# oriolfornes/ExplaiNN

Hardware: AMD Instinct MI355X
Metric: sequences/sec (fwd+bwd), 200bp one-hot, 300 units, batch 1024 (higher is better)
Workload: dtype f32

## Files before the change

### explainn_amd/csrc/convpool.hip

```cpp
#include <cstdlib>
#include <type_traits>

#include "common.h"

typedef __attribute__((ext_vector_type(8))) __bf16 cbf16x8;
typedef float cf32x16 __attribute__((ext_vector_type(16)));
typedef uint32_t cu32x4 __attribute__((ext_vector_type(4)));

template <int KS, int UT> struct cpm_state {
    cu32x4 Wr[UT][KS][3];
    cf32x16 acc[3][UT];
    float best[UT][16];
    uint32_t arg[UT][16];
    cu32x4 bop[3][KS];
    uint32_t xs[3], nx[2];
    uint32_t gw[4], mw[3];
    uint32_t smask[UT][16];
    uint32_t so, so4;
    uint32_t r1, r5;
};
struct cpm_args {
    const uint32_t* pk2; const uint32_t* nmask; float* ext; uint8_t* idx;
    int n, Bs, PW, NW, t0, b, kh; uint32_t tbase;
    uint32_t row1, row5;
    __amdgpu_buffer_rsrc_t rext, ridx;
};
__device__ __forceinline__ constexpr int cpm_role(int i) { return i == 0 ? 0 : ((i & 1) ? 1 : 2); }

template <int KS, int UT>
__device__ __forceinline__ void cpm_fetch(cpm_state<KS, UT>& S, const cpm_args& A, int w) {
    const int p0 = POOLW * w, wi = p0 >> 4, ni = p0 >> 5;
#pragma unroll
    for (int i = 0; i < 4; ++i) S.gw[i] = A.pk2[(size_t)min(wi + i, A.PW - 1) * A.Bs + A.b];
#pragma unroll
    for (int i = 0; i < 3; ++i) S.mw[i] = A.nmask[(size_t)min(ni + i, A.NW - 1) * A.Bs + A.b];
}
template <int KS, int UT>
__device__ __forceinline__ void cpm_window_words(cpm_state<KS, UT>& S, const cpm_args& A, int w) {
    const int p0 = POOLW * w;
    const int sh = (p0 & 15) * 2, nsh = p0 & 31;
    const uint32_t w0 = __funnelshift_r(S.gw[0], S.gw[1], sh), w1 = __funnelshift_r(S.gw[1], S.gw[2], sh),
                   w2 = __funnelshift_r(S.gw[2], S.gw[3], sh);
    S.xs[0] = __funnelshift_r(w0, w1, 4 * A.kh); S.xs[1] = __funnelshift_r(w1, w2, 4 * A.kh);
    S.xs[2] = w2 >> (4 * A.kh);
    const uint32_t nm0 = __funnelshift_r(S.mw[0], S.mw[1], nsh), nm1 = __funnelshift_r(S.mw[1], S.mw[2], nsh);
    S.nx[0] = __funnelshift_r(nm0, nm1, 2 * A.kh); S.nx[1] = nm1 >> (2 * A.kh);
    cpm_fetch(S, A, w + 1);
}
template <int KS, int UT, int I, int KSI, int BUF>
__device__ __forceinline__ void cpm_operand(cpm_state<KS, UT>& S, const cpm_args& A) {
    typedef __attribute__((address_space(3))) cu32x4 lds_u4;
    typedef __attribute__((address_space(3))) char lds_char;
    constexpr int off = 2 * I + 8 * KSI, wd = off >> 5, o = off & 31;
    constexpr int noff = I + 4 * KSI, nwd = noff >> 5, no = noff & 31;
    uint32_t cs, ns;
    if constexpr (o + 4 <= 32) {
        if constexpr (o >= 4) cs = S.xs[wd] >> (o - 4); else cs = S.xs[wd] << (4 - o);
    } else {
        cs = __funnelshift_r(S.xs[wd], S.xs[wd + 1], o) << 4;
    }
    if constexpr (no + 2 <= 32) {
        if constexpr (no >= 8) ns = S.nx[nwd] >> (no - 8); else ns = S.nx[nwd] << (8 - no);
    } else {
        ns = __funnelshift_r(S.nx[nwd], S.nx[nwd + 1], no) << 8;
    }
    const uint32_t a = ((cs & 0xF0u) | A.tbase) | (ns & 0x300u);
    S.bop[BUF][KSI] = *reinterpret_cast<const lds_u4*>((const lds_char*)(size_t)a);
}
template <int KS, int UT, bool IDX, int PI, int ROLE>
__device__ __forceinline__ void cpm_update_cmp(cpm_state<KS, UT>& S, int t, int r, unsigned long long& gt) {
    const float v = S.acc[ROLE][t][r];
    if (PI == 0) {
        S.best[t][r] = v;
    } else if (IDX) {
        asm volatile("v_cmp_gt_f32_e64 %0, %1, %2" : "=s"(gt) : "v"(v), "v"(S.best[t][r]));
    } else {
        float bv = S.best[t][r];
        asm volatile("v_max_f32 %0, %0, %1" : "+v"(bv) : "v"(v));
        S.best[t][r] = bv;
    }
}
template <int KS, int UT, bool IDX, int PI, int ROLE>
__device__ __forceinline__ void cpm_update_sel(cpm_state<KS, UT>& S, int t, int r, unsigned long long gt) {
    if (PI != 0 && IDX) {
        const float v = S.acc[ROLE][t][r];
        float bv = S.best[t][r];
        uint32_t av = PI == 1 ? 0u : S.arg[t][r];
        asm volatile("v_cndmask_b32_e64 %0, %0, %1, %2" : "+v"(bv) : "v"(v), "s"(gt));
        if (PI == 1) asm volatile("v_cndmask_b32_e64 %0, 0, 1, %1" : "=v"(av) : "s"(gt));
        else asm volatile("v_cndmask_b32_e64 %0, %0, %1, %2" : "+v"(av) : "n"(PI), "s"(gt));
        S.best[t][r] = bv; S.arg[t][r] = av;
    }
}
template <int KS, int UT, bool IDX, int PI, int ROLE>
__device__ __forceinline__ void cpm_update(cpm_state<KS, UT>& S, int t, int r) {
    unsigned long long gt = 0;
    cpm_update_cmp<KS, UT, IDX, PI, ROLE>(S, t, r, gt);
    asm volatile("s_nop 1");
    cpm_update_sel<KS, UT, IDX, PI, ROLE>(S, t, r, gt);
}
template <int KS, int UT, bool IDX>
__device__ __forceinline__ void cpm_store(cpm_state<KS, UT>& S, const cpm_args& A, int t, int r) {
    __builtin_amdgcn_raw_buffer_store_b32(__float_as_uint(S.best[t][r]) ^ S.smask[t][r], A.rext, (int)S.so4, 0, 0);
    if (IDX) __builtin_amdgcn_raw_buffer_store_b8((uint8_t)S.arg[t][r], A.ridx, (int)S.so, 0, 0);
    if (IDX) S.so += (r & 3) == 3 ? S.r5 : S.r1;
    S.so4 += (r & 3) == 3 ? 4u * S.r5 : 4u * S.r1;
}
#define CPM_OOB 0xFFFFFF00u

__device__ __forceinline__ uint32_t cpm_store_origin(const cpm_args& A, int w) {
    return (uint32_t)((4 * A.kh * A.n + w) * A.Bs + A.b);
}

#define CPM_GUARD 2
template <int K0, int K1, typename F>
__device__ __forceinline__ void cpm_static_for(F&& f) {
    if constexpr (K0 < K1) {
        f(std::integral_constant<int, K0>{});
        cpm_static_for<K0 + 1, K1>(f);
    }
}
template <int KS, int UT, int I> struct cpm_sched {
    static constexpr int NM = 3 * KS * UT;
    static constexpr int T0 = (UT + 1) / 2;
    static constexpr int NX = I == 6 ? 1 : 0, NG = KS, NE = 16 * UT;
    static constexpr int NS0 = I == 0 ? 16 * T0 : 0;
    static constexpr int NS1 = I == 1 ? 16 * (UT - T0) : 0;
    static constexpr int WX = 12, WG = 5, WE = (I == 1) ? 1 : 3, WS = 9;
    static constexpr int TOT = NX * WX + NG * WG + NE * WE + (NS0 + NS1) * WS;
    static constexpr int NU = NX + NG + NS1 + NE + NS0;
    static constexpr int E0 = NX + NG + NS1;
    static constexpr int weight(int k) {
        return k < NX ? WX : k < NX + NG ? WG : k < E0 ? WS : k < E0 + NE ? WE : WS;
    }
    static constexpr int slot(int k) {
        int cum = 0;
        for (int j = 0; j < k; ++j) cum += weight(j);
        int sl = (cum * NM) / (TOT > 0 ? TOT : 1);
        if (k >= E0 && sl < CPM_GUARD) sl = CPM_GUARD < NM ? CPM_GUARD : NM - 1;
        return sl < NM ? sl : NM - 1;
    }
    static constexpr int first_unit(int m) {
        int k = 0;
        while (k < NU && slot(k) < m) ++k;
        return k;
    }
};

template <int KS, int UT, bool IDX, int I>
__device__ __forceinline__ void cpm_position(cpm_state<KS, UT>& S, const cpm_args& A, int w) {
    typedef cpm_sched<KS, UT, I> SC;
    constexpr int NM = SC::NM;
    constexpr int RM = cpm_role(I), RN = cpm_role((I + 1) % POOLW), RP = cpm_role((I + POOLW - 1) % POOLW);
    constexpr int PI = (I + POOLW - 1) % POOLW;
    unsigned long long gt[3] = {0, 0, 0};
    cpm_static_for<0, NM>([&](auto mc) {
        constexpr int m = decltype(mc)::value;
        constexpr int pc = 2 - m / (KS * UT), ks = (m / UT) % KS, t = m % UT;
        if constexpr (m < UT)
            asm volatile("v_mfma_f32_32x32x16_bf16 %0, %1, %2, 0"
                         : "=&v"(S.acc[RM][t]) : "a"(S.Wr[t][ks][pc]), "a"(S.bop[RM][ks]));
        else
            asm volatile("v_mfma_f32_32x32x16_bf16 %0, %1, %2, %0"
                         : "+v"(S.acc[RM][t]) : "a"(S.Wr[t][ks][pc]), "a"(S.bop[RM][ks]));
        cpm_static_for<SC::first_unit(m), SC::first_unit(m + 1)>([&](auto kc) {
            constexpr int k = decltype(kc)::value;
            if constexpr (k < SC::NX) {
                cpm_window_words(S, A, w + 1);
            } else if constexpr (k < SC::NX + SC::NG) {
                cpm_operand<KS, UT, (I + 1) % POOLW, k - SC::NX, RN>(S, A);
            } else if constexpr (k < SC::E0) {
                constexpr int e = k - SC::NX - SC::NG;
                cpm_store<KS, UT, IDX>(S, A, SC::T0 + e / 16, e % 16);
            } else if constexpr (k < SC::E0 + SC::NE) {
                constexpr int e = k - SC::E0;
                if constexpr (e == 0 && NM <= CPM_GUARD) asm volatile("s_nop 15\n\ts_nop 15" ::: "memory");
                cpm_update_cmp<KS, UT, IDX, PI, RP>(S, e / 16, e % 16, gt[e % 3]);
                if constexpr (e > 1) cpm_update_sel<KS, UT, IDX, PI, RP>(S, (e - 2) / 16, (e - 2) % 16, gt[(e - 2) % 3]);
                if constexpr (e == SC::NE - 1) {
                    cpm_update_sel<KS, UT, IDX, PI, RP>(S, (e - 1) / 16, (e - 1) % 16, gt[(e - 1) % 3]);
                    cpm_update_sel<KS, UT, IDX, PI, RP>(S, e / 16, e % 16, gt[e % 3]);
                }
            } else {
                constexpr int e = k - SC::E0 - SC::NE;
                cpm_store<KS, UT, IDX>(S, A, e / 16, e % 16);
            }
        });
        __builtin_amdgcn_sched_barrier(0);
    });
}

template <int KS, int UT, bool IDX>
__device__ __forceinline__ void cpm_window(cpm_state<KS, UT>& S, const cpm_args& A, int w) {
    cpm_position<KS, UT, IDX, 0>(S, A, w);
    cpm_position<KS, UT, IDX, 1>(S, A, w);
    cpm_position<KS, UT, IDX, 2>(S, A, w);
    cpm_position<KS, UT, IDX, 3>(S, A, w);
    cpm_position<KS, UT, IDX, 4>(S, A, w);
    cpm_position<KS, UT, IDX, 5>(S, A, w);
    cpm_position<KS, UT, IDX, 6>(S, A, w);
}

template <int KS, int UT>
__device__ __forceinline__ void cpm_load_fragments(cpm_state<KS, UT>& S, const cu32x4* wsrc) {
    cpm_static_for<0, UT * KS * 3>([&S, wsrc](auto ic) {
        constexpr int i = decltype(ic)::value;
        cu32x4& dst = S.Wr[i / (KS * 3)][(i / 3) % KS][i % 3];
        const cu32x4* src = wsrc + 64 * i;
        asm volatile("global_load_dwordx4 %0, %1, off" : "=a"(dst) : "v"(src));
    });
}

struct cpm_bn1_args {
    const unsigned long long* bm; double* G; double* m;
    const float* conv_w; const float* conv_b; const float* g1; const float* b1;
    float* rm; float* rv; int64_t* nbt;
    float* alpha; float* shift; double* mug; double* sig1; double* Gw;
    int* ticket; int* flags;
    int naux, nz;
    int U, U4, k, B, L, Lp;
};
typedef __attribute__((address_space(1))) unsigned long long bn1_gu64;
typedef __attribute__((address_space(1))) int bn1_gi32;
template <int KS, int UT> struct bn1_cfg {
    static constexpr bool big = UT == 2 && KS >= 2;
    static constexpr int TQ = big ? 16 : 4;
    static constexpr int CH = big ? 40 : 12;
};
#define BN1_NU 2
#define BN1_SPIN_TICKS 10000000ull

__device__ __forceinline__ void bn1_store(double* p, double v) {
    __hip_atomic_store((bn1_gu64*)p, (unsigned long long)__double_as_longlong(v), __ATOMIC_RELAXED,
                       __HIP_MEMORY_SCOPE_AGENT);
}

template <int BN1_TQ>
__device__ __forceinline__ void bn1_moments_job(const cpm_bn1_args& X, int job, int lane) {
    const int d = job >> 2, a = job & 3;
    const int NT = (X.B + 63) / 64, Lo = X.L - X.k + 1, K4 = 4 * X.k;
    const size_t plane = (size_t)NT * X.Lp;
    const unsigned long long* __restrict__ m0 = X.bm + (size_t)a * plane;
    long long carry[4] = {0, 0, 0, 0}, plo[4] = {0, 0, 0, 0}, phi[4] = {0, 0, 0, 0};
    const int jlo = lane - 1, jhi = lane + Lo - 1;
    for (int qb = 0; qb < X.L; qb += 64) {
        const int q = qb + lane;
        int c[4] = {0, 0, 0, 0};
        if (q + d < X.L) {
            for (int t0 = 0; t0 < NT; t0 += BN1_TQ) {
                unsigned long long x0[BN1_TQ], x1[4][BN1_TQ];
#pragma unroll
                for (int i = 0; i < BN1_TQ; ++i) {
                    const size_t o = (size_t)min(t0 + i, NT - 1) * X.Lp + q;
                    x0[i] = m0[o];
#pragma unroll
                    for (int a2 = 0; a2 < 4; ++a2) x1[a2][i] = X.bm[a2 * plane + d + o];
                }
#pragma unroll
                for (int i = 0; i < BN1_TQ; ++i)
#pragma unroll
                    for (int a2 = 0; a2 < 4; ++a2) c[a2] += (t0 + i < NT) ? __popcll(x0[i] & x1[a2][i]) : 0;
            }
        }
#pragma unroll
        for (int a2 = 0; a2 < 4; ++a2) {
            int v = c[a2];
#pragma unroll
            for (int off = 1; off < 64; off <<= 1) {
                const int y = __shfl_up(v, off, 64);
                if (lane >= off) v += y;
            }
            const int vlo = __shfl(v, jlo & 63, 64), vhi = __shfl(v, jhi & 63, 64);
            if (jlo >= qb && jlo < qb + 64) plo[a2] = carry[a2] + vlo;
            if (jhi >= qb && jhi < qb + 64) phi[a2] = carry[a2] + vhi;
            carry[a2] += __shfl(v, 63, 64);
        }
    }
    const int j = lane;
    if (j < X.k - d) {
#pragma unroll
        for (int a2 = 0; a2 < 4; ++a2) {
            const long long sj = phi[a2] - plo[a2];
            const double v = (double)sj / ((double)X.B * (double)Lo);
            const int row = a * X.k + j, col = a2 * X.k + j + d;
            bn1_store(X.G + (size_t)row * K4 + col, v);
            bn1_store(X.G + (size_t)col * K4 + row, v);
            if (row == col) bn1_store(X.m + row, v);
        }
    }
}

template <int CH>
__device__ __forceinline__ void bn1_fold_units(const cpm_bn1_args& X, const int (&us)[BN1_NU], int nu, int lane) {
    const int K4 = 4 * X.k, Lo = X.L - X.k + 1;
    const int i0 = lane, i1 = lane + 64;
    const int c0i = min(i0, K4 - 1), c1i = min(i1, K4 - 1);
    float wl[BN1_NU][2];
#pragma unroll
    for (int uu = 0; uu < BN1_NU; ++uu) {
        const int u = min(us[uu], X.U - 1);
        wl[uu][0] = X.conv_w[(size_t)u * K4 + c0i];
        wl[uu][1] = X.conv_w[(size_t)u * K4 + c1i];
    }
    const double m0 = X.m[c0i], m1 = X.m[c1i];
    double ge[BN1_NU][2], go[BN1_NU][2];
#pragma unroll
    for (int uu = 0; uu < BN1_NU; ++uu) ge[uu][0] = ge[uu][1] = go[uu][0] = go[uu][1] = 0;
    for (int cb = 0; cb < K4; cb += CH) {
        double gv[CH][2];
#pragma unroll
        for (int cc = 0; cc < CH; ++cc) {
            const int c = min(cb + cc, K4 - 1);
            gv[cc][0] = X.G[(size_t)c * K4 + c0i];
            gv[cc][1] = X.G[(size_t)c * K4 + c1i];
        }
#pragma unroll
        for (int cc = 0; cc < CH; cc += 2) {
            const int c = cb + cc;
            if (c < K4) {
#pragma unroll
                for (int uu = 0; uu < BN1_NU; ++uu) {
                    const float we = __int_as_float(__builtin_amdgcn_readlane(
                        __float_as_int(c < 64 ? wl[uu][0] : wl[uu][1]), c & 63));
                    const float wo = __int_as_float(__builtin_amdgcn_readlane(
                        __float_as_int(c + 1 < 64 ? wl[uu][0] : wl[uu][1]), (c + 1) & 63));
#pragma unroll
                    for (int h = 0; h < 2; ++h) {
                        ge[uu][h] = fma(gv[cc][h], (double)we, ge[uu][h]);
                        go[uu][h] = fma(gv[cc + 1][h], (double)wo, go[uu][h]);
                    }
                }
            }
        }
    }
#pragma unroll
    for (int uu = 0; uu < BN1_NU; ++uu) {
        if (uu >= nu) break;
        const int u = us[uu];
        if (u >= X.U) {
            if (lane == 0) { X.alpha[u] = 0.f; X.shift[u] = 0.f; }
            continue;
        }
        double mu_p[2] = {0, 0}, q_p[2] = {0, 0};
#pragma unroll
        for (int h = 0; h < 2; ++h) {
            const int i = h ? i1 : i0;
            const double gw = ge[uu][h] + go[uu][h];
            if (i < K4) {
                X.Gw[(size_t)u * K4 + i] = gw;
                mu_p[h] = fma((double)wl[uu][h], h ? m1 : m0, mu_p[h]);
                q_p[h] = fma((double)wl[uu][h], gw, q_p[h]);
            }
        }
        const double mu = wave_sum_d(mu_p[0]) + wave_sum_d(mu_p[1]);
        const double wGw = wave_sum_d(q_p[0]) + wave_sum_d(q_p[1]);
        if (lane == 0)
            bn1_fold_finish(mu, wGw, u, X.g1[u], X.b1[u], X.conv_b[u], X.rm[u], X.rv[u], X.B, Lo, X.alpha,
                            X.shift, X.mug, X.sig1, X.rm, X.rv, X.nbt);
    }
}

template <int KS, int UT>
__device__ __forceinline__ void cpm_bn1(const cpm_bn1_args& X, int id, int lane) {
    for (int job = id; job < 4 * X.k; job += X.naux) bn1_moments_job<bn1_cfg<KS, UT>::TQ>(X, job, lane);
    asm volatile("s_waitcnt vmcnt(0)" ::: "memory");
    if (lane == 0) __hip_atomic_fetch_add((bn1_gi32*)X.ticket, 1, __ATOMIC_RELAXED, __HIP_MEMORY_SCOPE_AGENT);
    const unsigned long long t0 = wall_clock64();
    while (__builtin_amdgcn_readfirstlane(
               __hip_atomic_load((bn1_gi32*)X.ticket, __ATOMIC_RELAXED, __HIP_MEMORY_SCOPE_AGENT)) < X.naux) {
        if (wall_clock64() - t0 > BN1_SPIN_TICKS) {
            if (lane == 0)
                __hip_atomic_fetch_or((bn1_gi32*)X.flags, EXPLAINN_FLAG_BN1_TIMEOUT, __ATOMIC_RELAXED,
                                      __HIP_MEMORY_SCOPE_AGENT);
            return;
        }
        __builtin_amdgcn_s_sleep(2);
    }
    __builtin_amdgcn_fence(__ATOMIC_ACQUIRE, "agent");
    for (int u0 = id; u0 < X.U4; u0 += BN1_NU * X.naux) {
        int us[BN1_NU], nu = 0;
#pragma unroll
        for (int uu = 0; uu < BN1_NU; ++uu) {
            us[uu] = u0 + uu * X.naux;
            if (us[uu] < X.U4) nu = uu + 1;
        }
        bn1_fold_units<bn1_cfg<KS, UT>::CH>(X, us, nu, lane);
    }
}

template <int KS, int UT, bool IDX>
__global__ __launch_bounds__(64, (UT == 1 && KS <= 5) ? 2 : 1) void conv_pool_mm_kernel(
    const uint32_t* __restrict__ pk2, const uint32_t* __restrict__ nmask,
    const cu32x4* __restrict__ Wf, const cu32x4* __restrict__ Wsg,
    float* __restrict__ ext, uint8_t* __restrict__ idx, int n, int Bs, int PW, int NW, int wper,
    const cpm_bn1_args bn1) {
    __shared__ __attribute__((aligned(1024))) cu32x4 oh[64];
    typedef __attribute__((address_space(3))) char lds_char;
    const int lane = threadIdx.x;
    if constexpr (IDX) {
        if ((int)blockIdx.z < bn1.nz) {
            const int id = ((int)blockIdx.z * (int)gridDim.y + (int)blockIdx.y) * (int)gridDim.x + (int)blockIdx.x;
            if (id < bn1.naux) cpm_bn1<KS, UT>(bn1, id, lane);
            return;
        }
    }
    STAMP(0);
    {
        const int c4 = lane & 15, nb = lane >> 4;
        uint32_t r[4] = {0u, 0u, 0u, 0u};
#pragma unroll
        for (int h = 0; h < 2; ++h) {
            const int cde = (c4 >> (2 * h)) & 3;
            const uint32_t one = ((nb >> h) & 1) ? 0u : 0x3F80u;
#pragma unroll
            for (int q = 0; q < 4; ++q)
                if (q == 2 * h + (cde >> 1)) r[q] = one << (16 * (cde & 1));
        }
        oh[lane] = cu32x4{r[0], r[1], r[2], r[3]};
    }
    cpm_state<KS, UT> S;
    cpm_args A;
    A.pk2 = pk2; A.nmask = nmask; A.ext = ext; A.idx = idx; A.n = n; A.Bs = Bs; A.PW = PW; A.NW = NW;
    A.t0 = blockIdx.y * UT; A.b = blockIdx.x * 32 + (lane & 31); A.kh = lane >> 5;
    A.tbase = (uint32_t)(size_t)(const lds_char*)oh;
    A.row1 = (uint32_t)(n * Bs); A.row5 = 5u * A.row1;
    {
        const size_t row0 = (size_t)32 * A.t0 * n * Bs;
        const int span = __builtin_amdgcn_readfirstlane(32 * UT * n * Bs);
        auto uniform = [](auto* q) {
            const unsigned long long v = reinterpret_cast<unsigned long long>(q);
            const unsigned lo = __builtin_amdgcn_readfirstlane((unsigned)v), hi = __builtin_amdgcn_readfirstlane((unsigned)(v >> 32));
            return reinterpret_cast<decltype(q)>(((unsigned long long)hi << 32) | lo);
        };
        A.rext = __builtin_amdgcn_make_buffer_rsrc(uniform(ext + row0), 0, 4 * span, 0x00020000);
        A.ridx = __builtin_amdgcn_make_buffer_rsrc(uniform(idx + row0), 0, span, 0x00020000);
    }
    const int wbeg = (IDX ? (int)blockIdx.z - bn1.nz : (int)blockIdx.z) * wper, wend = min(n, wbeg + wper);
    if (wbeg >= wend) return;
    cpm_load_fragments(S, Wf + (size_t)A.t0 * KS * 3 * 64 + lane);
    cpm_fetch(S, A, wbeg);
    {
        const cu32x4* ssrc = Wsg + ((size_t)A.t0 * 2 + A.kh) * 4;
#pragma unroll
        for (int t = 0; t < UT; ++t)
#pragma unroll
            for (int q = 0; q < 4; ++q) {
                const cu32x4 v = ssrc[t * 8 + q];
#pragma unroll
                for (int i = 0; i < 4; ++i) S.smask[t][4 * q + i] = v[i];
            }
    }
    asm volatile("s_waitcnt vmcnt(0)" ::: "memory");
    __syncthreads();
    STAMP(1);
    cpm_window_words(S, A, wbeg);
    cpm_static_for<0, KS>([&](auto kc) { cpm_operand<KS, UT, 0, decltype(kc)::value, 0>(S, A); });
    STAMP(2);
#pragma unroll 1
    for (int w = wbeg; w < wend; ++w) {
        const bool first = w == wbeg;
        S.so = first ? CPM_OOB : cpm_store_origin(A, w - 1);
        S.so4 = first ? CPM_OOB : 4u * S.so;
        S.r1 = first ? 0u : A.row1; S.r5 = first ? 0u : A.row5;
        cpm_window<KS, UT, IDX>(S, A, w);
        if (first) STAMP(3);
    }
    STAMP(4);
    __builtin_amdgcn_sched_barrier(0);
    asm volatile("s_nop 15\n\ts_nop 15\n\ts_nop 15" ::: "memory");
    __builtin_amdgcn_sched_barrier(0);
#pragma unroll
    for (int t = 0; t < UT; ++t)
#pragma unroll
        for (int r = 0; r < 16; ++r) cpm_update<KS, UT, IDX, POOLW - 1, 2>(S, t, r);
    S.so = cpm_store_origin(A, wend - 1);
    S.so4 = 4u * S.so;
    S.r1 = A.row1; S.r5 = A.row5;
#pragma unroll
    for (int t = 0; t < UT; ++t)
#pragma unroll
        for (int r = 0; r < 16; ++r) cpm_store<KS, UT, IDX>(S, A, t, r);
    STAMP(5);
}

static int conv_pool_mm_ut(const explainn_ctx* c) {
    if (const char* e = getenv("EXPLAINN_CPM_UT")) { const int v = atoi(e); if (v == 1 || (v == 2 && conv_ksteps(c->k) <= 5)) return v; }
    return conv_ut(c->k);
}

static int conv_pool_mm_parts(const explainn_ctx* c, int B, int ut) {
    if (const char* e = getenv("EXPLAINN_CPM_PARTS")) { const int v = atoi(e); if (v >= 1) return min(v, c->n); }
    const int groups = ut == 1 ? (c->U + 31) / 32 : conv_tiles_padded(c->U, c->k) / ut, sb = (B + 31) / 32;
    const int cols = groups * sb, slots = (ut == 1 && conv_ksteps(c->k) <= 5) ? 2048 : 1024;
    int best = 1;
    long best_cost = -1;
    for (int p = 1; p <= c->n; ++p) {
        const int wper = (c->n + p - 1) / p, np = (c->n + wper - 1) / wper;
        if (np != p) continue;
        const long rounds = ((long)cols * np + slots - 1) / slots;
        const long cost = rounds * (wper + 1);
        if (best_cost < 0 || cost < best_cost) { best_cost = cost; best = p; }
    }
    return best;
}

int conv_pool_bn1_workgroups(const explainn_ctx* c, int B) {
    if (const char* e = getenv("EXPLAINN_BN1_AUX")) return min(max(atoi(e), 0), 256);
    const int ut = conv_pool_mm_ut(c);
    const int parts = conv_pool_mm_parts(c, B, ut);
    const int wper = (c->n + parts - 1) / parts;
    const long blocks = (long)((B + 31) / 32) * (ut == 1 ? (c->U + 31) / 32 : conv_tiles_padded(c->U, c->k) / ut) *
                        ((c->n + wper - 1) / wper);
    const int slots = (ut == 1 && conv_ksteps(c->k) <= 5) ? 2048 : 1024;
    return blocks >= 768 && blocks <= slots && c->L <= 256 ? 8 * c->k : 0;
}

static int launch_conv_pool_mm(explainn_ctx* c, const explainn_params* p, int B, bool want_idx,
                               cpm_bn1_args* bn1, hipStream_t s) {
    const int ut = conv_pool_mm_ut(c);
    const int parts = conv_pool_mm_parts(c, B, ut);
    const int wper = (c->n + parts - 1) / parts;
    dim3 grid((B + 31) / 32, ut == 1 ? (c->U + 31) / 32 : conv_tiles_padded(c->U, c->k) / ut, (c->n + wper - 1) / wper);
    cpm_bn1_args none = {};
    if (bn1) {
        const int slice = (int)(grid.x * grid.y);
        bn1->nz = (bn1->naux + slice - 1) / slice;
        grid.z += bn1->nz;
    }
    const cpm_bn1_args& bn1v = bn1 ? *bn1 : none;
#define ARGS grid, dim3(64), 0, s, c->pk2, c->nmask, reinterpret_cast<const cu32x4*>(c->Wf), \
             reinterpret_cast<const cu32x4*>(c->Wsg), c->ext, c->idx, c->n, c->Bs, c->PW, c->NW, wper, bn1v
#define CALLKS(KSv, UTv)                                                                        \
    if (want_idx) hipLaunchKernelGGL((conv_pool_mm_kernel<KSv, UTv, true>), ARGS);              \
    else hipLaunchKernelGGL((conv_pool_mm_kernel<KSv, UTv, false>), ARGS);
#define CALLUT(KSv) if (ut == 2) { CALLKS(KSv, 2); } else { CALLKS(KSv, 1); }
    switch (conv_ksteps(c->k)) {
#ifndef CPM_ONLY5
        case 1: { CALLUT(1); } break;
        case 2: { CALLUT(2); } break;
        case 3: { CALLUT(3); } break;
        case 4: { CALLUT(4); } break;
        case 6: { CALLKS(6, 1); } break;
        case 7: { CALLKS(7, 1); } break;
        case 8: { CALLKS(8, 1); } break;
#endif
        case 5: { CALLUT(5); } break;
        default: explainn_set_error("kernel_size %d not instantiated (2..32)", c->k); return EXPLAINN_E_UNSUPPORTED;
    }
#undef CALLUT
#undef CALLKS
#undef ARGS
    LAUNCH_CHECK();
    return EXPLAINN_OK;
}

int launch_conv_pool(explainn_ctx* c, const explainn_params* p, int B, bool want_idx, hipStream_t s) {
    return launch_conv_pool_mm(c, p, B, want_idx, nullptr, s);
}

int launch_conv_pool_train(explainn_ctx* c, const explainn_params* p, int B, int naux, hipStream_t s) {
    cpm_bn1_args a = {c->bm, c->G, c->m, p->conv_w, p->conv_b, p->bn1_w, p->bn1_b, p->bn1_rm, p->bn1_rv,
                      p->bn1_nbt, c->alpha, c->shift, c->mug, c->sig1, c->Gw, c->bn1_ticket, c->flags,
                      naux, 0, c->U, c->U4, c->k, B, c->L, c->Lp};
    return launch_conv_pool_mm(c, p, B, true, &a, s);
}

__global__ __launch_bounds__(256) void conv_act_kernel(const uint8_t* __restrict__ codesT,
                                                       const float* __restrict__ Wt,
                                                       const float* __restrict__ alpha,
                                                       const float* __restrict__ shift,
                                                       float* __restrict__ acts, int U, int k,
                                                       int L, int Lo, int Bs) {
    extern __shared__ float4 Wsm[];
    uint8_t* cs = reinterpret_cast<uint8_t*>(Wsm + k * 5);
    const int b = blockIdx.x, quad = blockIdx.y;
    const float4* src = reinterpret_cast<const float4*>(Wt) + (size_t)quad * k * 5;
    for (int i = threadIdx.x; i < k * 5; i += 256) Wsm[i] = src[i];
    for (int p = threadIdx.x; p < L; p += 256) cs[p] = codesT[(size_t)p * Bs + b];
    __syncthreads();
    for (int p = threadIdx.x; p < Lo; p += 256) {
        float4 acc = make_float4(0.f, 0.f, 0.f, 0.f);
        for (int j = 0; j < k; ++j) {
            const float4 v = Wsm[j * 5 + cs[p + j]];
            acc.x += v.x; acc.y += v.y; acc.z += v.z; acc.w += v.w;
        }
        const float av[4] = {acc.x, acc.y, acc.z, acc.w};
#pragma unroll
        for (int uu = 0; uu < 4; ++uu) {
            const int u = quad * 4 + uu;
            if (u < U) acts[((size_t)b * U + u) * Lo + p] = qval(alpha[u], av[uu], shift[u]);
        }
    }
}

int launch_conv_act(explainn_ctx* c, int B, float* acts, hipStream_t s) {
    const size_t sm = (size_t)c->k * 5 * sizeof(float4) + ((c->L + 15) & ~15);
    hipLaunchKernelGGL(conv_act_kernel, dim3(B, c->Uq), dim3(256), sm, s, c->codesT, c->Wt, c->alpha,
                       c->shift, acts, c->U, c->k, c->L, c->Lo, c->Bs);
    LAUNCH_CHECK();
    return EXPLAINN_OK;
}
```

Measured before the change: 5.682 million.

## Split BN1 moment jobs finer and batch fold-unit reductions across lanes

Splits each BN1 moment job into two items covering half of the second-channel set, and batches several 64-position panels per item so the scans and shuffles are interleaved. This is meant to improve load balance across the auxiliary waves and expose more memory-level parallelism. The fold step now reduces all units' partial sums together with xor shuffles, prefetches per-unit scalar parameters in parallel across lanes, and finishes each unit on a separate lane instead of serially on lane 0. The tile sizes change, and STAMP timing hooks are inserted, which may add overhead if they are enabled.

Result: faster. 5.889 million, median of 6 (+3.6%).

```diff
diff --git a/explainn_amd/csrc/convpool.hip b/explainn_amd/csrc/convpool.hip
--- a/explainn_amd/csrc/convpool.hip
+++ b/explainn_amd/csrc/convpool.hip
@@ -222,10 +222,12 @@
 };
 typedef __attribute__((address_space(1))) unsigned long long bn1_gu64;
 typedef __attribute__((address_space(1))) int bn1_gi32;
+typedef __attribute__((address_space(1))) float bn1_gf32;
 template <int KS, int UT> struct bn1_cfg {
     static constexpr bool big = UT == 2 && KS >= 2;
-    static constexpr int TQ = big ? 16 : 4;
-    static constexpr int CH = big ? 40 : 12;
+    static constexpr int PQ = big ? 4 : 2;
+    static constexpr int TQ = big ? 6 : 3;
+    static constexpr int CH = big ? 38 : 12;
 };
 #define BN1_NU 2
 #define BN1_SPIN_TICKS 10000000ull
@@ -235,54 +237,78 @@
                        __HIP_MEMORY_SCOPE_AGENT);
 }
 
-template <int BN1_TQ>
-__device__ __forceinline__ void bn1_moments_job(const cpm_bn1_args& X, int job, int lane) {
-    const int d = job >> 2, a = job & 3;
+template <int TQ, int PQ>
+__device__ __forceinline__ void bn1_moments_item(const cpm_bn1_args& X, int item, int lane) {
+    const int d = item >> 3, a = (item >> 1) & 3, ab = (item & 1) * 2;
     const int NT = (X.B + 63) / 64, Lo = X.L - X.k + 1, K4 = 4 * X.k;
     const size_t plane = (size_t)NT * X.Lp;
     const unsigned long long* __restrict__ m0 = X.bm + (size_t)a * plane;
-    long long carry[4] = {0, 0, 0, 0}, plo[4] = {0, 0, 0, 0}, phi[4] = {0, 0, 0, 0};
-    const int jlo = lane - 1, jhi = lane + Lo - 1;
-    for (int qb = 0; qb < X.L; qb += 64) {
-        const int q = qb + lane;
-        int c[4] = {0, 0, 0, 0};
-        if (q + d < X.L) {
-            for (int t0 = 0; t0 < NT; t0 += BN1_TQ) {
-                unsigned long long x0[BN1_TQ], x1[4][BN1_TQ];
-#pragma unroll
-                for (int i = 0; i < BN1_TQ; ++i) {
-                    const size_t o = (size_t)min(t0 + i, NT - 1) * X.Lp + q;
-                    x0[i] = m0[o];
-#pragma unroll
-                    for (int a2 = 0; a2 < 4; ++a2) x1[a2][i] = X.bm[a2 * plane + d + o];
+    const unsigned long long* __restrict__ m1 = X.bm + (size_t)ab * plane + d;
+    long long carry[2] = {0, 0}, plo[2] = {0, 0}, phi[2] = {0, 0};
+    const int jhi = lane + Lo - 1;
+    const int pa = (Lo - 1) >> 6;
+    for (int p0 = 0; p0 * 64 < X.L; p0 += PQ) {
+        int c[PQ][2], qo[PQ];
+        bool ok[PQ];
+#pragma unroll
+        for (int p = 0; p < PQ; ++p) {
+            const int q = (p0 + p) * 64 + lane;
+            ok[p] = q + d < X.L;
+            qo[p] = min(q, X.L - 1 - d);
+            c[p][0] = c[p][1] = 0;
+        }
+        for (int t0 = 0; t0 < NT; t0 += TQ) {
+            unsigned long long x0[PQ][TQ], x1[PQ][2][TQ];
+#pragma unroll
+            for (int p = 0; p < PQ; ++p)
+#pragma unroll
+                for (int i = 0; i < TQ; ++i) {
+                    const size_t o = (size_t)min(t0 + i, NT - 1) * X.Lp + qo[p];
+                    x0[p][i] = m0[o];
+                    x1[p][0][i] = m1[o];
+                    x1[p][1][i] = m1[plane + o];
                 }
 #pragma unroll
-                for (int i = 0; i < BN1_TQ; ++i)
-#pragma unroll
-                    for (int a2 = 0; a2 < 4; ++a2) c[a2] += (t0 + i < NT) ? __popcll(x0[i] & x1[a2][i]) : 0;
+            for (int p = 0; p < PQ; ++p)
+#pragma unroll
+                for (int i = 0; i < TQ; ++i)
+#pragma unroll
+                    for (int s = 0; s < 2; ++s)
+                        c[p][s] += (ok[p] && t0 + i < NT) ? __popcll(x0[p][i] & x1[p][s][i]) : 0;
+        }
+        int v[PQ][2];
+#pragma unroll
+        for (int p = 0; p < PQ; ++p) { v[p][0] = c[p][0]; v[p][1] = c[p][1]; }
+#pragma unroll
+        for (int off = 1; off < 64; off <<= 1)
+#pragma unroll
+            for (int p = 0; p < PQ; ++p)
+#pragma unroll
+                for (int s = 0; s < 2; ++s) {
+                    const int y = __shfl_up(v[p][s], off, 64);
+                    if (lane >= off) v[p][s] += y;
+                }
+#pragma unroll
+        for (int p = 0; p < PQ; ++p) {
+            const int pg = p0 + p;
+#pragma unroll
+            for (int s = 0; s < 2; ++s) {
+                if (pg == 0) plo[s] = v[p][s] - c[p][s];
+                if (pg == pa || pg == pa + 1) {
+                    const int vhi = __shfl(v[p][s], jhi & 63, 64);
+                    if ((jhi >> 6) == pg) phi[s] = carry[s] + vhi;
+                }
+                carry[s] += __builtin_amdgcn_readlane(v[p][s], 63);
             }
-        }
-#pragma unroll
-        for (int a2 = 0; a2 < 4; ++a2) {
-            int v = c[a2];
-#pragma unroll
-            for (int off = 1; off < 64; off <<= 1) {
-                const int y = __shfl_up(v, off, 64);
-                if (lane >= off) v += y;
-            }
-            const int vlo = __shfl(v, jlo & 63, 64), vhi = __shfl(v, jhi & 63, 64);
-            if (jlo >= qb && jlo < qb + 64) plo[a2] = carry[a2] + vlo;
-            if (jhi >= qb && jhi < qb + 64) phi[a2] = carry[a2] + vhi;
-            carry[a2] += __shfl(v, 63, 64);
         }
     }
     const int j = lane;
     if (j < X.k - d) {
 #pragma unroll
-        for (int a2 = 0; a2 < 4; ++a2) {
-            const long long sj = phi[a2] - plo[a2];
+        for (int s = 0; s < 2; ++s) {
+            const long long sj = phi[s] - plo[s];
             const double v = (double)sj / ((double)X.B * (double)Lo);
-            const int row = a * X.k + j, col = a2 * X.k + j + d;
+            const int row = a * X.k + j, col = (ab + s) * X.k + j + d;
             bn1_store(X.G + (size_t)row * K4 + col, v);
             bn1_store(X.G + (size_t)col * K4 + row, v);
             if (row == col) bn1_store(X.m + row, v);
@@ -303,6 +329,26 @@
         wl[uu][1] = X.conv_w[(size_t)u * K4 + c1i];
     }
     const double m0 = X.m[c0i], m1 = X.m[c1i];
+    int ul = us[0];
+#pragma unroll
+    for (int uu = 1; uu < BN1_NU; ++uu) ul = lane == uu ? us[uu] : ul;
+    const bool fin = lane < nu && ul < X.U;
+    float par = 0.f;
+    static_assert(BN1_NU <= 8, "lane 8 uu + f: eight units' scalars fit the wave");
+    {
+        const int pu = lane >> 3, pf = lane & 7;
+        int uq = us[0];
+#pragma unroll
+        for (int uu = 1; uu < BN1_NU; ++uu) uq = pu == uu ? us[uu] : uq;
+        unsigned long long ps[5] = {(unsigned long long)X.g1, (unsigned long long)X.b1, (unsigned long long)X.conv_b,
+                                    (unsigned long long)X.rm, (unsigned long long)X.rv};
+#pragma unroll
+        for (int f = 0; f < 5; ++f) asm volatile("" : "+s"(ps[f]));
+        unsigned long long pa = ps[4];
+#pragma unroll
+        for (int f = 3; f >= 0; --f) pa = pf == f ? ps[f] : pa;
+        if (pu < nu && pf < 5 && uq < X.U) par = ((const bn1_gf32*)pa)[uq];
+    }
     double ge[BN1_NU][2], go[BN1_NU][2];
 #pragma unroll
     for (int uu = 0; uu < BN1_NU; ++uu) ge[uu][0] = ge[uu][1] = go[uu][0] = go[uu][1] = 0;
@@ -333,37 +379,61 @@
             }
         }
     }
+    STAMP(4);
+    double sm[BN1_NU][2][2];
 #pragma unroll
     for (int uu = 0; uu < BN1_NU; ++uu) {
-        if (uu >= nu) break;
-        const int u = us[uu];
-        if (u >= X.U) {
-            if (lane == 0) { X.alpha[u] = 0.f; X.shift[u] = 0.f; }
-            continue;
-        }
-        double mu_p[2] = {0, 0}, q_p[2] = {0, 0};
+        const bool live = uu < nu && us[uu] < X.U;
 #pragma unroll
         for (int h = 0; h < 2; ++h) {
             const int i = h ? i1 : i0;
             const double gw = ge[uu][h] + go[uu][h];
-            if (i < K4) {
-                X.Gw[(size_t)u * K4 + i] = gw;
-                mu_p[h] = fma((double)wl[uu][h], h ? m1 : m0, mu_p[h]);
-                q_p[h] = fma((double)wl[uu][h], gw, q_p[h]);
+            double mu_p = 0, q_p = 0;
+            if (live && i < K4) {
+                X.Gw[(size_t)us[uu] * K4 + i] = gw;
+                mu_p = fma((double)wl[uu][h], h ? m1 : m0, mu_p);
+                q_p = fma((double)wl[uu][h], gw, q_p);
             }
-        }
-        const double mu = wave_sum_d(mu_p[0]) + wave_sum_d(mu_p[1]);
-        const double wGw = wave_sum_d(q_p[0]) + wave_sum_d(q_p[1]);
-        if (lane == 0)
-            bn1_fold_finish(mu, wGw, u, X.g1[u], X.b1[u], X.conv_b[u], X.rm[u], X.rv[u], X.B, Lo, X.alpha,
-                            X.shift, X.mug, X.sig1, X.rm, X.rv, X.nbt);
-    }
+            sm[uu][0][h] = mu_p;
+            sm[uu][1][h] = q_p;
+        }
+    }
+#pragma unroll
+    for (int off = 32; off > 0; off >>= 1)
+#pragma unroll
+        for (int uu = 0; uu < BN1_NU; ++uu)
+#pragma unroll
+            for (int w = 0; w < 2; ++w)
+#pragma unroll
+                for (int h = 0; h < 2; ++h) sm[uu][w][h] += __shfl_xor(sm[uu][w][h], off, 64);
+    double mu = sm[0][0][0] + sm[0][0][1], wGw = sm[0][1][0] + sm[0][1][1];
+#pragma unroll
+    for (int uu = 1; uu < BN1_NU; ++uu) {
+        const double mu_u = sm[uu][0][0] + sm[uu][0][1], wGw_u = sm[uu][1][0] + sm[uu][1][1];
+        mu = lane == uu ? mu_u : mu;
+        wGw = lane == uu ? wGw_u : wGw;
+    }
+    float sc[5];
+#pragma unroll
+    for (int f = 0; f < 5; ++f) {
+        sc[f] = __int_as_float(__builtin_amdgcn_readlane(__float_as_int(par), f));
+#pragma unroll
+        for (int uu = 1; uu < BN1_NU; ++uu)
+            sc[f] = lane == uu ? __int_as_float(__builtin_amdgcn_readlane(__float_as_int(par), 8 * uu + f)) : sc[f];
+    }
+    if (fin)
+        bn1_fold_finish(mu, wGw, ul, sc[0], sc[1], sc[2], sc[3], sc[4], X.B, Lo, X.alpha, X.shift, X.mug, X.sig1,
+                        X.rm, X.rv, X.nbt);
+    else if (lane < nu) { X.alpha[ul] = 0.f; X.shift[ul] = 0.f; }
 }
 
 template <int KS, int UT>
 __device__ __forceinline__ void cpm_bn1(const cpm_bn1_args& X, int id, int lane) {
-    for (int job = id; job < 4 * X.k; job += X.naux) bn1_moments_job<bn1_cfg<KS, UT>::TQ>(X, job, lane);
+    typedef bn1_cfg<KS, UT> cfg;
+    STAMP(0);
+    for (int item = id; item < 8 * X.k; item += X.naux) bn1_moments_item<cfg::TQ, cfg::PQ>(X, item, lane);
     asm volatile("s_waitcnt vmcnt(0)" ::: "memory");
+    STAMP(1);
     if (lane == 0) __hip_atomic_fetch_add((bn1_gi32*)X.ticket, 1, __ATOMIC_RELAXED, __HIP_MEMORY_SCOPE_AGENT);
     const unsigned long long t0 = wall_clock64();
     while (__builtin_amdgcn_readfirstlane(
@@ -376,7 +446,9 @@
         }
         __builtin_amdgcn_s_sleep(2);
     }
+    STAMP(2);
     __builtin_amdgcn_fence(__ATOMIC_ACQUIRE, "agent");
+    STAMP(3);
     for (int u0 = id; u0 < X.U4; u0 += BN1_NU * X.naux) {
         int us[BN1_NU], nu = 0;
 #pragma unroll
@@ -384,8 +456,9 @@
             us[uu] = u0 + uu * X.naux;
             if (us[uu] < X.U4) nu = uu + 1;
         }
-        bn1_fold_units<bn1_cfg<KS, UT>::CH>(X, us, nu, lane);
-    }
+        bn1_fold_units<cfg::CH>(X, us, nu, lane);
+    }
+    STAMP(5);
 }
 
 template <int KS, int UT, bool IDX>
```
